# mjrgh/DCSExplorer

Measured on AMD Instinct MI355X. Metric: bit_exact_int16_pcm_samples_per_sec, higher is better.
Workload: dtype int16; 1 GPU; survey3_65536; gpu_max_hw_queues=4, samples_per_frame=240, frames_per_wave=8, wavefronts_per_launch=8192, arithmetic=ADSP-2105 1.15 fixed point, 32-bit integer intermediates, partition=range over streams, no collective, scale=1, inflight=1, frames_per_chunk=all, full=False

## Files before the change

### dcsexplorer_amd/csrc/dcs_common.h

```cpp
#pragma once
#include <stdint.h>
#include <stddef.h>
#include "../../include/dcs_hip.h"

#define DCS_CB94_TOTAL   940
#define DCS_TRIE94_MAX   64
#define DCS_TRIE93_MAX   128

struct DcsLdsTables
{
    uint16_t cb94[DCS_CB94_TOTAL];
    uint16_t fast93[256];
    uint16_t trie93[DCS_TRIE93_MAX];
    uint16_t bandBits93a[64];
    uint16_t scaleCb93a[80];
    uint8_t  inputs93a[24];
    uint16_t raw94[20];
    uint32_t band94[72];
    uint16_t scale64[64];
    uint8_t  padDecode_[8];
    uint16_t cbInfo[8];
    uint16_t xlat94[48];
    uint8_t  preAdj94[32];
    uint16_t scaleMant[4];
    uint8_t  pad_[8];
};
#define DCS_LDS_DECODE_BYTES 3424
#define DCS_B94_RAW      (1u << 21)
#define DCS_B94_ZERO     (1u << 22)
#define DCS_B94_STOP     (1u << 23)
#define DCS_B94_FATAL    (1u << 24)
#define DCS_B94_TYPE0    51

#define DCS_LANE_CONSTS 24
#define DCS_K94_PRE   0
#define DCS_K94_TWB   8
#define DCS_K94_OVLA  22
#define DCS_K94_OVLB  23
#define DCS_K93_TWB   0
#define DCS_K93_OVL   15

struct DcsDevTables
{
    DcsLdsTables lds;
    uint32_t lane94[64][DCS_LANE_CONSTS];
    uint32_t lane93[64][DCS_LANE_CONSTS];
    uint16_t fast94[256];
    uint16_t trie94[DCS_TRIE94_MAX];
    uint16_t pair93a[2048];
    uint16_t fftCoef[256];
    uint16_t ovlCoef[16];
    int32_t  twA[8][4];
    uint8_t  multi94[6][1 << 10];
};
#define DCS_IDX_MULTI_BITS 10
#define DCS_IDX_MULTI_SAMPLES 4

const DcsDevTables &dcsTables();

int dcsFrameScaleV(const uint16_t *vol, uint16_t *mixMul, const uint8_t *counted, int nch);

#define DCS_POOL_DW_PER_FRAME 56
#define DCS_POOL_DW_MIN       320
#define DCS_MAX_FRAME_BITS    4480

#ifdef __cplusplus
static inline
#ifdef __HIPCC__
__host__ __device__
#endif
uint32_t dcsPoolDwords(uint64_t streamOff, uint32_t hdrLen, uint32_t bitOff, uint32_t nBits)
{
    const uint32_t inDword = static_cast<uint32_t>(((streamOff + 2 + hdrLen) * 8 + bitOff) & 31);
    return (inDword + nBits + 31) / 32 + 3;
}
#endif

#ifdef __cplusplus
static inline
#ifdef __HIPCC__
__host__ __device__
#endif
constexpr uint32_t dcsPoolCapacity(int fpw)
{
    return static_cast<uint32_t>(fpw * DCS_POOL_DW_PER_FRAME > DCS_POOL_DW_MIN ? fpw * DCS_POOL_DW_PER_FRAME : DCS_POOL_DW_MIN);
}
#endif

#define DCS_SLOT_HALO      0x01u
#define DCS_SLOT_EXT_TAIL  0x02u
#define DCS_SLOT_EXPORT    0x04u
#define DCS_SLOT_IMPORT    0x08u
#define DCS_SLOT_KEEP_TAIL 0x10u
#define DCS_SLOT_EMPTY     0x80u
#define DCS_NO_PREV_SLOT   0xFFu

struct DcsSlot
{
    uint32_t job;
    uint8_t  prevSlot;
    uint8_t  flags;
    uint8_t  nSrc;
    uint8_t  shiftXform;
    uint32_t firstSrc;
    uint32_t prevJob;
    uint32_t runStartDw;
    uint16_t runNDw;
// ... 177 lines not shown
```

### dcsexplorer_amd/csrc/dcs_decode_chunk.inc.h

```cpp
    DCS_STAMP(1);

    struct { uint32_t job; uint32_t prevSlot, flags, nSrc, shiftXform; uint32_t firstSrc, prevJob, poolOff, bpl; } slot;
    uint32_t exportNext;
    uint4 pd0, pd1, phdr;
    uint2 pd2;
    {
        uint4 *scratch = reinterpret_cast<uint4 *>(L.pool());
        static_assert(kHeadVec * 16 <= poolDwords(FPW) * 4, "the package head fits in the bit pool");
        if (lane < kHeadVec)
            scratch[lane] = phead0;
        if (kHeadLoads > 1 && lane + 64 < kHeadVec)
            scratch[lane + 64] = phead1;
        waveSync();
        const uint4 *sp5 = scratch + 5 * s;
        const uint4 s0 = sp5[0];
        pd0 = sp5[1]; pd1 = sp5[2];
        const uint4 d2v = sp5[3];
        pd2 = make_uint2(d2v.x, d2v.y);
        phdr = sp5[4];
        waveSync();
        slot.job = s0.x;
        slot.prevSlot = s0.y & 0xFFu; slot.flags = (s0.y >> 8) & 0xFFu; slot.nSrc = (s0.y >> 16) & 0xFFu; slot.shiftXform = s0.y >> 24;
        slot.firstSrc = s0.z; slot.prevJob = s0.w;
        slot.poolOff = d2v.z & 0xFFFFu;
        slot.bpl = (d2v.z >> 16) & 0xFFu;
        const unsigned long long exportSlots = __ballot(lane < FPW && !(slot.flags & DCS_SLOT_EMPTY) && (slot.flags & DCS_SLOT_EXPORT) != 0);
        exportNext = static_cast<uint32_t>(__builtin_amdgcn_readlane(static_cast<int>(d2v.w), exportSlots != 0 ? static_cast<int>(__builtin_ctzll(exportSlots)) : 0));
    }

    const int firstXform = __builtin_amdgcn_readfirstlane(static_cast<int>(slot.shiftXform >> 4)) == DCS_XFORM_94 ? DCS_XFORM_94 : DCS_XFORM_93;
    if (PASS == 0 || firstXform != constsXform)
    {
        constsXform = firstXform;
        loadLaneConsts(a.tables, lane, constsXform, C);
    }
#pragma unroll
    for (int t = 0 ; t < kPoolPieces ; ++t)
    {
        const int i = lane * 4 + 256 * t;
        const bool in = i < imgDw;
        if (i < poolDwords(FPW))
            ldsWrite4(L.pool() + i, in ? pimg[t].x : 0u, in ? pimg[t].y : 0u, in ? pimg[t].z : 0u, in ? pimg[t].w : 0u);
    }

    const bool live = !(slot.flags & DCS_SLOT_EMPTY);
    struct { uint32_t firstSrc; int nSrc; int volShift; int xform; uint32_t prev; } job;
    job.firstSrc = slot.firstSrc; job.nSrc = slot.nSrc; job.volShift = slot.shiftXform & 15;
    job.xform = slot.shiftXform >> 4; job.prev = slot.prevJob;

    uint32_t err = 0;
    {
        uint32_t *pool = L.pool();
        const DcsLdsTables *T = L.tables();
        uint16_t *row = L.row(s);
        const uint32_t *blobW = reinterpret_cast<const uint32_t *>(a.blob);
        const uint32_t blobWords = static_cast<uint32_t>((a.blobLen + 3) >> 2);
        const int myNSrc = live ? job.nSrc : 0;

        auto unpackRound = [&](auto r0tag, const int r)
        {
            constexpr bool R0 = decltype(r0tag)::value;
            const bool has = r < myNSrc;
            const uint4 *sdp = reinterpret_cast<const uint4 *>(&a.srcs[has ? job.firstSrc + r : 0]);
            uint4 d0 = make_uint4(0, 0, 0, 0), d1 = d0;
            uint2 d2 = make_uint2(0, 0);
            uint2 sp = make_uint2(0, 0);
            const int bplSlot = slot.bpl;
            if (R0)
            {
                if (has) { d0 = pd0; d1 = pd1; d2 = pd2; sp = psplit; }
            }
            else if (has) { d0 = sdp[0]; d1 = sdp[1]; d2 = *reinterpret_cast<const uint2 *>(sdp + 2); }
            const uint64_t streamOff = static_cast<uint64_t>(d0.x) | (static_cast<uint64_t>(d0.y) << 32);
            const uint32_t mixMul = d0.z & 0xFFFFu;
            const int format = static_cast<int>((d0.z >> 16) & 0xFFu);
            const int hdrLen = has ? static_cast<int>(d0.z >> 24) : 16;
            const uint32_t bitOff = d0.w;
            const uint32_t nBits = d1.x & 0xFFFFu, hdrBits = d1.x >> 16;
            const int nBands = static_cast<int>((d2.y >> 16) & 0xFFu);
            const uint32_t flags = d2.y >> 24;
// ... 120 lines not shown
                    Q.nb = max((q == SUB - 1 ? nbEnd : nextBase) - myBase, 0);
                    if (SUB == 16)
                    {
                        const bool mid = format >= DCS_FMT_94_T0 && q == SUB - 1 && myBase == 15 && (sp.y & (DCS_SPLIT_MID15 << 16)) != 0;
                        const bool nextMid = __shfl(static_cast<int>(mid), lane + FPW) != 0;
                        Q.midStart = mid;
                        Q.midStraddle = mid && (sp.y & (DCS_MID15_STRADDLE << 16)) != 0;
                        Q.midEnd = q == SUB - 2 && nextMid;
                        if (Q.midEnd)
                            Q.nb = 16 - myBase;
                    }
                }
                else
                {
                    const int bpl = max((nb16 + SUB - 1) / SUB, 1);
                    if (format == DCS_FMT_93A_T1)
                    {
                        Q.bandBase = min(q * bpl, nb16);
                        Q.nb = min(max(nb16 - Q.bandBase, 0), bpl);
                    }
                    else
                    {
                        Q.bandBase = dcsLaneFirstBand(format, q, bpl, nb16);
                        Q.nb = (q == SUB - 1 ? nb16 : dcsLaneFirstBand(format, q + 1, bpl, nb16)) - Q.bandBase;
                    }
                }
                if (q != 0 && Q.nb != 0)
                {
                    if (!R0)
                        sp = reinterpret_cast<const uint2 *>(sdp)[5 + Q.bandBase - 1];
                    const uint32_t sp0 = sp.x, sp1 = sp.y;
                    relBits = sp0 & 0x7FFFu;
                    Q.prv = sp0 >> 16;
                    Q.prvDelta = sp1 & 0xFFFFu;
                    const uint32_t st = sp1 >> 16;
                    Q.outIdx = static_cast<int>(st & 0x1FFu);
                    Q.subType = static_cast<int>((st >> 9) & 3u);
                    Q.reuse = (st & 0x800u) != 0;
                    Q.first = false;
                }
            }
            const uint32_t inPool = static_cast<uint32_t>(bitPos & 31) + relBits;
            const uint32_t *brAt = pool + (ok ? off + (inPool >> 5) : 0u);
            const int brBit = static_cast<int>(inPool & 31);

            if (R0) DCS_STAMP(12);
            const bool is94 = ok && format >= DCS_FMT_94_T0;
            const bool is93a = ok && format == DCS_FMT_93A_T1 && Q.nb != 0 && !(Q.bandBase != 0 && Q.reuse);
            const bool is93 = ok && format < DCS_FMT_93A_T1;
            if (__any(is94))
            {
                BR94 br;
                br.init(brAt, brBit);
                err |= unpack94<R0, BR94, SUB>(T, row, br, Q, format, mixMul, is94, stamp);
            }
            BR93 br;
            br.init(brAt, brBit);
            if (__any(is93))
                err |= unpack93<R0, BR93>(T, row, br, Q, format, mixMul, is93, stamp);
            if (is93a)
            {
                constexpr bool kSpreadTail = SUB == 16 && !R0;
                const int end = Q.bandBase + Q.nb;
                const int end2 = (!R0 && SUB != 16 && end >= 16 && nBands > 16) ? nBands : end;
                const int prv0 = Q.bandBase == 0 ? 0x1A : sx16(Q.prv), out0 = Q.bandBase == 0 ? 0 : Q.outIdx;
                const int hb0 = static_cast<int>(Q.h0 & 0xFFu);
                if (pairTableInLds(FPW))
                    err |= unpack93a<R0, BR93>(T, row, br, hb0, mixMul, reinterpret_cast<const uint16_t *>(smem + ldsBytes(FPW) - 4096),
                                         Q.bandBase, end2, prv0, out0);
                else
                    err |= unpack93a<R0, BR93>(T, row, br, hb0, mixMul, a.tables->pair93a, Q.bandBase, end2, prv0, out0);
                if (kSpreadTail && pairTableInLds(FPW) && q < 2 && 16 + q < nBands)
                {
                    const uint32_t r0 = q == 0 ? Q.t0 : Q.t2, r1 = q == 0 ? Q.t1 : Q.t3;
                    if (!((r1 >> 16) & 0x800u))
                    {
                        const uint32_t inPool2 = static_cast<uint32_t>(bitPos & 31) + (r0 & 0xFFFFu);
                        BR93 br2;
                        br2.init(pool + off + (inPool2 >> 5), static_cast<int>(inPool2 & 31));
                        err |= unpack93a<R0, BR93>(T, row, br2, hb0, mixMul, reinterpret_cast<const uint16_t *>(smem + ldsBytes(FPW) - 4096),
                                             16 + q, 17 + q, sx16(r0 >> 16), static_cast<int>((r1 >> 16) & 0x1FFu));
                    }
                }
            }
            waveSync();
        };

        {
            if (__any(myNSrc > 0))
                unpackRound(std::true_type{}, 0);
            for (int r = 1 ; __any(r < myNSrc) ; ++r)
                unpackRound(std::false_type{}, r);
        }

        DCS_STAMP(4);
        if (__any(err != 0))
        {
#pragma unroll
            for (int m = FPW ; m < 64 ; m <<= 1)
                err |= __shfl_xor(err, m);
        }
        if (live && q == 0)
        {
            if (job.xform == DCS_XFORM_93)
                dcMagnitude93(row);
            if (!(slot.flags & DCS_SLOT_HALO) && a.err != nullptr)
                a.err[slot.job] = err;
// ... 191 lines not shown
```

### dcsexplorer_amd/csrc/dcs_kernels.hip.h

```cpp
#pragma once
#include <hip/hip_runtime.h>
#include <type_traits>
#include <cstddef>
#include "dcs_common.h"

namespace dcsk {

struct Stamper
{
#ifdef DCS_STAMPS
    unsigned long long *p;
#ifdef DCS_STAMPS_REALTIME
    __device__ __forceinline__ void operator()(int k) const { if (p != nullptr) p[k] = __builtin_amdgcn_s_memrealtime(); }
#else
    __device__ __forceinline__ void operator()(int k) const { if (p != nullptr) p[k] = __builtin_amdgcn_s_memtime(); }
#endif
#else
    __device__ __forceinline__ void operator()(int) const { }
#endif
};
#define DCS_STAMP(k) stamp(k)

__device__ __forceinline__ unsigned long long handoffWord(uint32_t epoch, uint32_t who, uint32_t payload)
{
    return (static_cast<unsigned long long>(epoch) << 33) | (static_cast<unsigned long long>(who) << 32) | payload;
}
__device__ __forceinline__ bool handoffMeets(unsigned long long old, uint32_t epoch, uint32_t whoWanted)
{
    return static_cast<uint32_t>(old >> 32) == ((epoch << 1) | whoWanted);
}
constexpr int kWavesPerBlock = 4;
#ifndef DCS_ROW_BYTES
#define DCS_ROW_BYTES 528
#endif
constexpr int kRowBytes = DCS_ROW_BYTES;

__host__ __device__ constexpr int poolDwords(int fpw) { return static_cast<int>(dcsPoolCapacity(fpw)); }
__host__ __device__ constexpr int subLanes(int fpw) { return 64 / fpw; }

__host__ __device__ constexpr int waveLdsBytes(int fpw) { return fpw * kRowBytes + (fpw + 1) * 32 + poolDwords(fpw) * 4; }
__host__ __device__ constexpr bool pairTableInLds(int fpw) { return fpw <= 8; }
__host__ __device__ constexpr int ldsBytes(int fpw)
{
    return DCS_LDS_DECODE_BYTES + kWavesPerBlock * waveLdsBytes(fpw) + (pairTableInLds(fpw) ? 4096 : 0);
}

__device__ __forceinline__ int sx16(uint32_t v) { return static_cast<int>(static_cast<int16_t>(v)); }

__device__ __forceinline__ int sat16(int v) { return min(max(v, -32768), 32767); }

__device__ __forceinline__ uint32_t prodSS(int a, int b) { return static_cast<uint32_t>(__mul24(a, b)) << 1; }

__device__ __forceinline__ int roundHi(uint32_t mr, int lastProdUndoubled)
{
    mr += 0x8000u;
    if ((lastProdUndoubled & 0x7FFF) == 0x4000)
        mr &= ~0x10000u;
    return static_cast<int>(mr) >> 16;
}

__device__ __forceinline__ void rotate(int are, int aim, int c, int s, int &tre, int &tim)
{
    const int p1 = __mul24(are, c), p2 = __mul24(aim, s);
    tre = roundHi(static_cast<uint32_t>(p1 - p2) << 1, p2);
    const int q1 = __mul24(aim, c), q2 = __mul24(are, s);
    tim = roundHi(static_cast<uint32_t>(q1 + q2) << 1, q2);
}

__device__ __forceinline__ int calcExp32(uint32_t x)
{
    const uint32_t y = (static_cast<int>(x) < 0) ? ~x : x;
    int n = (y == 0) ? 32 : __clz(static_cast<int>(y));
    n -= 1;
    if (n > 31) n = 31;
    return -n;
}

typedef const uint32_t __attribute__((address_space(3))) *LdsDwordPtr;
struct BitReader
{
    static constexpr bool kDirect = false;
    uint32_t pa;
    uint32_t hi, lo;
    int negpos;

    __device__ __forceinline__ void init(const uint32_t *pool, int bitInDword)
    {
        hi = 0;
        lo = pool[0];
        pa = static_cast<uint32_t>(reinterpret_cast<uintptr_t>((LdsDwordPtr)(pool + 1)));
        negpos = 0;
        skip(bitInDword);
    }
    __device__ __forceinline__ uint32_t cur() const { return __builtin_amdgcn_alignbit(hi, lo, static_cast<uint32_t>(negpos)); }
    __device__ __forceinline__ uint32_t peek(int n) const { return cur() >> (32 - n); }
    __device__ __forceinline__ uint32_t prefetch() const { return *reinterpret_cast<LdsDwordPtr>(static_cast<uintptr_t>(pa)); }
    __device__ __forceinline__ void skip(int n, uint32_t ahead)
    {
        negpos -= n;
        const bool refill = negpos < 0;
        hi = refill ? lo : hi;
        lo = refill ? ahead : lo;
        const uint32_t sign = static_cast<uint32_t>(negpos) >> 31;
        asm("v_lshl_add_u32 %0, %1, 2, %0" : "+v"(pa) : "v"(sign));
        negpos &= 31;
    }
    __device__ __forceinline__ void skipTight(uint32_t n, uint32_t ahead)
    {
        uint32_t t;
        asm("v_sub_co_u32 %3, vcc, %3, %5\n\t"
            "v_cndmask_b32 %0, %0, %1, vcc\n\t"
            "v_cndmask_b32 %1, %1, %6, vcc\n\t"
            "v_lshrrev_b32 %4, 31, %3\n\t"
            "v_lshl_add_u32 %2, %4, 2, %2\n\t"
            "v_and_b32 %3, 31, %3"
            : "+v"(hi), "+v"(lo), "+v"(pa), "+v"(negpos), "=&v"(t)
            : "v"(n), "v"(ahead)
            : "vcc");
    }
    __device__ __forceinline__ void skip(int n) { skip(n, prefetch()); }
    __device__ __forceinline__ uint32_t get(int n) { const uint32_t v = peek(n); skip(n); return v; }
    __device__ __forceinline__ uint32_t bitAddr() const { return (pa - 4u) * 8u - static_cast<uint32_t>(negpos); }
    __device__ __forceinline__ void initAt(uint32_t bits)
    {
        init((const uint32_t *)reinterpret_cast<LdsDwordPtr>(static_cast<uintptr_t>((bits >> 5) << 2)), static_cast<int>(bits & 31u));
    }
};

struct DirectReader
{
    static constexpr bool kDirect = true;
    uint32_t bp;

    __device__ __forceinline__ void init(const uint32_t *pool, int bitInDword)
    {
        bp = static_cast<uint32_t>(reinterpret_cast<uintptr_t>((LdsDwordPtr)pool)) * 8u + static_cast<uint32_t>(bitInDword) - 1u;
    }
    __device__ __forceinline__ uint32_t cur() const
    {
        const LdsDwordPtr w = reinterpret_cast<LdsDwordPtr>(static_cast<uintptr_t>((bp >> 3) & ~3u));
        return __builtin_amdgcn_alignbit(w[0], w[1], ~bp);
    }
    __device__ __forceinline__ uint32_t peek(int n) const { return cur() >> (32 - n); }
    __device__ __forceinline__ uint32_t prefetch() const { return 0u; }
    __device__ __forceinline__ void skip(int n) { bp += static_cast<uint32_t>(n); }
    __device__ __forceinline__ void skip(int n, uint32_t) { skip(n); }
    __device__ __forceinline__ void skipTight(uint32_t n, uint32_t) { bp += n; }
    __device__ __forceinline__ uint32_t get(int n) { const uint32_t v = peek(n); skip(n); return v; }
    __device__ __forceinline__ uint32_t bitAddr() const { return bp + 1u; }
    __device__ __forceinline__ void initAt(uint32_t bits) { bp = bits - 1u; }
};

template <class BR>
__device__ __forceinline__ int readVlc(BR &br, const uint16_t *fast, const uint16_t *trie)
{
    uint32_t e = fast[br.peek(8)];
    if (e & 0x8000)
    {
        br.skip(static_cast<int>((e >> 8) & 0xF));
        return static_cast<int>(e & 0xFF);
    }
    br.skip(8);
    uint32_t w = br.cur();
    int n = 0;
    do
    {
        e = trie[e + (w >> 31)];
        w <<= 1;
        ++n;
    }
    while (!(e & 0x8000) && n < 24);
    br.skip(n);
    return static_cast<int>(e & 0xFF);
}

template <int FPW>
struct Lds
{
    unsigned char *tab;
    unsigned char *base;
    unsigned char *poolBase;
    __device__ __forceinline__ const DcsLdsTables *tables() const { return reinterpret_cast<const DcsLdsTables *>(tab); }
    __device__ __forceinline__ uint16_t *row(int s) const { return reinterpret_cast<uint16_t *>(base + s * kRowBytes); }
    __device__ __forceinline__ uint16_t *tails() const { return reinterpret_cast<uint16_t *>(base + FPW * kRowBytes); }
    __device__ __forceinline__ uint32_t *pool() const { return reinterpret_cast<uint32_t *>(poolBase); }
};

struct Quarter
{
    uint32_t h0, h1, h2, h3;
    uint32_t t0, t1, t2, t3;
    int bandBase;
    int nb;
    int outIdx;
    uint32_t preAdj;
    uint32_t prv, prvDelta;
    int subType;
    bool reuse, first;
    bool midEnd, midStart, midStraddle;
};

__device__ __forceinline__ int byteOf(uint32_t w0, uint32_t w1, uint32_t w2, uint32_t w3, int b)
{
    const int i = b >> 2;
    const uint32_t lo = (i & 1) ? w1 : w0, hi = (i & 1) ? w3 : w2;
    const uint32_t w = (i & 2) ? hi : lo;
    return static_cast<int>((w >> (8 * (b & 3))) & 0xFFu);
}

__device__ __forceinline__ int mul24(int a, int b)
{
    int r;
    asm("v_mul_i32_i24 %0, %1, %2" : "=v"(r) : "v"(a), "v"(b));
    return r;
}

template <bool FIRST>
__device__ __forceinline__ void mixAdd(uint16_t *cell, int scaledProduct, uint32_t mixMul)
{
    uint32_t t, acc;
    asm("v_mul_i32_i24_sdwa %0, sext(%1), %2 dst_sel:DWORD dst_unused:UNUSED_PAD src0_sel:WORD_0 src1_sel:DWORD"
        : "=v"(t) : "v"(scaledProduct), "v"(mixMul));
    asm("v_add_u32_sdwa %0, %1, %2 dst_sel:DWORD dst_unused:UNUSED_PAD src0_sel:DWORD src1_sel:WORD_0"
        : "=v"(acc) : "v"(t), "v"(scaledProduct));
    if (!FIRST)
        acc += static_cast<uint32_t>(*cell) << 16;
    *cell = static_cast<uint16_t>(acc >> 16);
}
typedef uint16_t __attribute__((address_space(3))) *LdsWordPtr;
template <bool FIRST>
__device__ __forceinline__ void mixAddAt(uint32_t cellAddr, int scaledProduct, uint32_t mixMul)
{
    const LdsWordPtr cell = reinterpret_cast<LdsWordPtr>(static_cast<uintptr_t>(cellAddr));
    uint32_t t, acc;
    asm("v_mul_i32_i24_sdwa %0, sext(%1), %2 dst_sel:DWORD dst_unused:UNUSED_PAD src0_sel:WORD_0 src1_sel:DWORD"
        : "=v"(t) : "v"(scaledProduct), "v"(mixMul));
    asm("v_add_u32_sdwa %0, %1, %2 dst_sel:DWORD dst_unused:UNUSED_PAD src0_sel:DWORD src1_sel:WORD_0"
        : "=v"(acc) : "v"(t), "v"(scaledProduct));
// ... 5 lines not shown
__device__ __forceinline__ uint32_t mixAddCarry(uint16_t *cell, int scaledProduct, uint32_t mixMul, uint32_t addLow)
{
    uint32_t t, acc;
    asm("v_mul_i32_i24_sdwa %0, sext(%1), %2 dst_sel:DWORD dst_unused:UNUSED_PAD src0_sel:WORD_0 src1_sel:DWORD"
        : "=v"(t) : "v"(scaledProduct), "v"(mixMul));
    asm("v_add_u32_sdwa %0, %1, %2 dst_sel:DWORD dst_unused:UNUSED_PAD src0_sel:DWORD src1_sel:WORD_0"
        : "=v"(acc) : "v"(t), "v"(addLow));
    if (!FIRST)
        acc += static_cast<uint32_t>(*cell) << 16;
    *cell = static_cast<uint16_t>(acc >> 16);
    return acc;
}
template <bool FIRST>
__device__ __forceinline__ uint32_t mixAddCarryAt(uint32_t cellAddr, int scaledProduct, uint32_t mixMul, uint32_t addLow)
{
    const LdsWordPtr cell = reinterpret_cast<LdsWordPtr>(static_cast<uintptr_t>(cellAddr));
    uint32_t t, acc;
    asm("v_mul_i32_i24_sdwa %0, sext(%1), %2 dst_sel:DWORD dst_unused:UNUSED_PAD src0_sel:WORD_0 src1_sel:DWORD"
        : "=v"(t) : "v"(scaledProduct), "v"(mixMul));
    asm("v_add_u32_sdwa %0, %1, %2 dst_sel:DWORD dst_unused:UNUSED_PAD src0_sel:DWORD src1_sel:WORD_0"
        : "=v"(acc) : "v"(t), "v"(addLow));
    if (!FIRST)
        acc += static_cast<uint32_t>(*cell) << 16;
    *cell = static_cast<uint16_t>(acc >> 16);
    return acc;
}
__device__ __forceinline__ int mulLowWord(uint32_t x, int y)
{
    int r;
    asm("v_mul_i32_i24_sdwa %0, sext(%1), %2 dst_sel:DWORD dst_unused:UNUSED_PAD src0_sel:WORD_0 src1_sel:DWORD" : "=v"(r) : "v"(x), "v"(y));
    return r;
}
__device__ __forceinline__ void mixSub(uint16_t *cell, int scaledProduct, uint32_t mixMul)
{
    const uint32_t s = static_cast<uint32_t>(scaledProduct) & 0xFFFFu;
    const uint32_t c = (s + static_cast<uint32_t>(__mul24(sx16(s), static_cast<int>(mixMul)))) >> 16;
    *cell = static_cast<uint16_t>(*cell - c);
}

__device__ __forceinline__ uint32_t scaleFactor(const DcsLdsTables *T, int code)
{
    return T->scale64[code & 63];
}

__device__ __forceinline__ void dcFixup(uint16_t *row, uint32_t saved1)
{
    const int delta = sat16(sx16(row[1]) - sx16(saved1));
    row[0] = static_cast<uint16_t>(sat16(delta + sx16(row[0])));
    row[1] = static_cast<uint16_t>(saved1);
}

constexpr int kDummyWord = 256;

template <bool FIRST, class BR, int SUB>
__device__ uint32_t unpack94(const DcsLdsTables *T, uint16_t *row, BR &br, const Quarter &Q,
                             int format, uint32_t mixMul, bool has, const Stamper &stamp)
{
    const bool type1 = format != DCS_FMT_94_T0;
    uint32_t err = 0;
    int nb = has ? Q.nb : 0;
    const int b1 = Q.bandBase + nb;
    const int before = Q.bandBase <= 0 ? 0 : Q.bandBase == 1 ? 7 : 15 + 16 * (Q.bandBase - 2);
    const int upTo = b1 <= 0 ? 0 : b1 == 1 ? 7 : b1 >= 16 ? 255 : 15 + 16 * (b1 - 2);
    const int midAdvance = 16 - (Q.midStraddle ? 1 + static_cast<int>((Q.h3 >> 30) & 1u) : 0);
    int outIdx = min(Q.outIdx, 256 - ((SUB == 16 && Q.midStart) ? midAdvance : upTo - before));
    bool valid = true;
    const bool owner = has && Q.bandBase == 0;
    const uint32_t saved1 = (owner && !FIRST) ? row[1] : 0u;

    stamp(8);
    int k = 0;
    const int keyLim = type1 ? 16 : 17;
    uint32_t cell = static_cast<uint32_t>(reinterpret_cast<uintptr_t>((LdsWordPtr)row)) + 2u * static_cast<uint32_t>(outIdx);
    uint32_t cellEnd = cell;
    uint32_t cellStart = cell;
    uint32_t startBits = 0;
    const uint16_t *book = T->cb94;
    int shPeek = 0, shIdx = 0, scale = 0;
    uint32_t incSh = 1;
    uint32_t valOff = 0, valWidth = 8;
    for (int round = 0 ; ; ++round)
    {
        if (SUB == 16 && Q.midEnd && cell > cellEnd)
            cellEnd = cell;
        if (cell > cellEnd)
        {
            cell -= 1u << incSh;
            if (valid)
            {
                BR r2;
                r2.initAt(startBits);
                uint32_t c2 = cellStart;
                while (c2 + (1u << incSh) < cellEnd)
                {
                    const uint32_t e = book[r2.cur() >> shIdx];
                    r2.skip(static_cast<int>((e >> 8) & 0x1F));
                    const uint32_t step = e >> 13;
                    if (step == 1)
                        mixSub((uint16_t *)reinterpret_cast<LdsWordPtr>(static_cast<uintptr_t>(c2)),
                               mul24(static_cast<int>(static_cast<int8_t>(e & 0xFF)), scale), mixMul);
                    c2 += step << incSh;
                }
            }
            valid = false; err |= DCS_FRAME_STOP;
            cellEnd = cell;
        }
        const bool start = cell == cellEnd && k < nb;
        if (!__any(start || cell < cellEnd))
            break;
        if (start)
        {
            const int band = Q.bandBase + k;
            ++k;
            const int hb = byteOf(Q.h0, Q.h1, Q.h2, Q.h3, band) & 0x7F;
            const int code0 = byteOf(Q.t0, Q.t1, Q.t2, Q.t3, band);
            const int cls = band < 3 ? 0 : band < 6 ? 17 : 34;
            const int key = min(code0, keyLim) + (type1 ? cls : DCS_B94_TYPE0);
            const uint32_t e = T->band94[key];
            const int count0 = band < 2 ? 7 + band : band == 15 ? 32 : 16;
            const uint32_t strided = (static_cast<uint32_t>(hb) >> 6) & 1u;
            const uint32_t count = static_cast<uint32_t>(count0) >> strided;
            incSh = 1u + strided;
            const int pre = (type1 && band < 3) ? static_cast<int>((Q.preAdj >> (4 * band)) & 15u) : 0;
            scale = static_cast<int>(scaleFactor(T, hb + pre + static_cast<int>(e >> 25)));
            book = reinterpret_cast<const uint16_t *>(T) + (e & 0x7FFu);
            shPeek = static_cast<int>((e >> 11) & 31u);
            shIdx = static_cast<int>((e >> 16) & 31u);
            const bool isRaw = (e & DCS_B94_RAW) != 0;
            valOff = isRaw ? static_cast<uint32_t>(shPeek) : 0u;
            valWidth = isRaw ? 32u - static_cast<uint32_t>(shPeek) : 8u;
            const bool zeroBand = (e & DCS_B94_ZERO) != 0, fatal = (e & DCS_B94_FATAL) != 0;
            uint32_t i = (e & (DCS_B94_ZERO | DCS_B94_FATAL)) == 0 ? count : 0u;
            if (SUB == 16 && band == 15 && i != 0)
            {
                if (Q.midEnd) i = count - (count >> 1);
                if (Q.midStart) i = (count >> 1) - (Q.midStraddle ? 1u : 0u);
            }
            cell += zeroBand ? 2u * count : 0u;
            if (fatal)
            {
                err |= DCS_FRAME_FATAL | DCS_FRAME_STOP;
                nb = 0;
            }
            if (!valid)
                scale = 0;
            cellStart = cell;
            cellEnd = cell + (i << incSh);
            startBits = br.bitAddr();
        }

        if (round == 0) stamp(9);
        const uint32_t roundLen = round == 0 ? 7u : round == 1 ? 9u : 16u;
        const uint32_t roundEnd = min(cellEnd, cell + (roundLen << incSh));
        if (cell < roundEnd)
        {
            do
            {
                const uint32_t ahead = br.prefetch();
                const uint32_t w = br.cur();
                const uint32_t e = book[w >> shIdx];
                const int v = __builtin_amdgcn_sbfe(__builtin_amdgcn_perm(w, e, 0x07060100u), valOff, valWidth);
                const uint32_t step = e >> 13;
                br.skipTight((e >> 8) & 0x1Fu, ahead);
// ... 704 lines not shown
    for (int r = 0 ; r < 16 ; ++r)
        x[r] = y[r];
    DCS_XSTAMP(10);
    DCS_PACE_STEP(1);
    stageB<false, 8, 4>(x, C.k + DCS_K93_TWB, R);
    stageB<false, 4, 3>(x, C.k + DCS_K93_TWB + 1, R);
    DCS_PACE_STEP(2);
    stageB<false, 2, 2>(x, C.k + DCS_K93_TWB + 3, R);
    stageB<false, 1, 1>(x, C.k + DCS_K93_TWB + 7, R);
    DCS_XSTAMP(11);
    if (__any(P.shiftPair != 0))
    {
#pragma unroll
        for (int r = 0 ; r < 16 ; ++r)
            x[r] = pkAshr(x[r], P.shiftPair);
    }
}

#ifndef DCS_CPW2_SCHED
#define DCS_CPW2_SCHED 1
#endif
struct PaceSchedule { int entry; bool steps; int levels; };
__host__ __device__ constexpr PaceSchedule paceSchedule(int cpw, int pass)
{
    if (cpw == 1)
        return { 3, true, kPaceSteps };
#if DCS_CPW2_SCHED == 0
    return pass == 0 ? PaceSchedule{ 3, false, kPaceSteps } : PaceSchedule{ 3, true, 2 | (1 << 2) | (0 << 4) };
#elif DCS_CPW2_SCHED == 1
    return pass == 0 ? PaceSchedule{ 3, false, kPaceSteps } : PaceSchedule{ 2, true, 1 | (1 << 2) | (0 << 4) };
#elif DCS_CPW2_SCHED == 2
    return pass == 0 ? PaceSchedule{ 3, true, 3 | (3 << 2) | (2 << 4) } : PaceSchedule{ 2, true, 1 | (1 << 2) | (0 << 4) };
#else
    return pass == 0 ? PaceSchedule{ 3, true, 3 | (2 << 2) | (2 << 4) } : PaceSchedule{ 1, true, 1 | (0 << 2) | (0 << 4) };
#endif
}

template <int FPW, int CPW = 1>
#ifndef DCS_MIN_WAVES
#define DCS_MIN_WAVES 4
#endif
__global__ void __launch_bounds__(64 * kWavesPerBlock, DCS_MIN_WAVES)
dcsDecodeKernel(uint8_t *kPackages, const DcsDevTables *kTables, uint32_t kNChunks, uint32_t kFlags, uint32_t kEpoch, uint32_t kNJobs,
                int16_t *kPcm, unsigned long long *kHandoff, uint32_t *kErr, int16_t *kTailsOut,
                const uint8_t *kBlob, uint64_t kBlobLen, const DcsSrcDesc *kSrcs, const int16_t *kTailsIn, unsigned long long *kDebug)
{
    DcsKernelArgs a;
    a.blob = kBlob; a.blobLen = kBlobLen; a.srcs = kSrcs; a.packages = kPackages; a.nChunks = kNChunks; a.nJobs = kNJobs;
    a.pcm = kPcm; a.err = kErr; a.tailsIn = kTailsIn; a.tailsOut = kTailsOut; a.tables = kTables; a.debug = kDebug;
    a.handoff = kHandoff; a.epoch = kEpoch; a.flags = kFlags;
    extern __shared__ __attribute__((aligned(16))) unsigned char smem[];
    const int wave = static_cast<int>(threadIdx.x) >> 6;
    const int lane = static_cast<int>(threadIdx.x) & 63;
    constexpr int kPoolBytes = poolDwords(FPW) * 4, kTileBytes = FPW * kRowBytes + (FPW + 1) * 32;
    static_assert(kPoolBytes % 16 == 0 && kWavesPerBlock * kTileBytes >= 8192, "LDS layout");
    const Lds<FPW> L{ smem, smem + DCS_LDS_DECODE_BYTES + kWavesPerBlock * kPoolBytes + wave * kTileBytes,
                      smem + DCS_LDS_DECODE_BYTES + wave * kPoolBytes };
    uint32_t blk = blockIdx.x;
    if (a.flags & DCS_BATCH_XCD_RANGES)
        blk = (blk & 7u) * (gridDim.x >> 3) + (blk >> 3);
    static_assert(CPW == 1 || CPW == 2, "one or two chunks per wavefront");
    const uint32_t wv = blk * kWavesPerBlock + static_cast<uint32_t>(wave);
    const uint32_t nFirst = CPW == 2 ? (a.nChunks + 1u) >> 1 : a.nChunks;
    auto stamperOf = [&](uint32_t chunk, bool valid)
    {
#ifdef DCS_STAMPS
        return Stamper{ (lane == 0 && a.debug != nullptr && valid) ? a.debug + static_cast<size_t>(chunk) * 16 : nullptr };
#else
        return Stamper{};
#endif
    };
    {
        const Stamper stamp = stamperOf(wv, wv < nFirst);
        DCS_STAMP(0);
    }
    const bool pacedLaunch = (a.flags & DCS_BATCH_PACED) != 0;
    const bool paced = pacedLaunch && blockIdx.x + ((a.flags >> DCS_BATCH_CUS8_SHIFT) & 0xFFu) * 32u >= gridDim.x;
    if (pacedLaunch) __builtin_amdgcn_s_setprio(3);
    constexpr int SUB = subLanes(FPW);
#ifndef DCS_DIRECT_MAX_FPW
#define DCS_DIRECT_MAX_FPW 4
#endif
    using BR94 = typename std::conditional<(FPW <= DCS_DIRECT_MAX_FPW), DirectReader, BitReader>::type;
    using BR93 = DirectReader;
    static_assert(SUB * FPW == 64 && SUB <= 16, "every lane unpacks; a frame has at most 16 split lanes");
    const int s = lane % FPW;
    const int q = lane / FPW;
    const bool unpacker = q < SUB;

    const uint32_t layout = (a.flags >> DCS_BATCH_IMG_SHIFT) & DCS_BATCH_IMG_MASK;
    const int imgDw = static_cast<int>(dcsPkgImgDw(layout));
    const bool split4 = (layout & DCS_PKG_SPLIT4) != 0;
    const uint32_t offPool = split4 ? dcsPkgOffPool(FPW, DCS_PKG_SPLIT4) : dcsPkgOffPool(FPW, 0);
    constexpr int kHeadVec = FPW * 5, kHeadLoads = (kHeadVec + 63) / 64;
    static_assert(kHeadLoads <= 2, "package head: two 16-byte loads per lane at most");
    uint4 phead0, phead1 = make_uint4(0, 0, 0, 0);
    uint2 psplit;
    constexpr int kPoolPieces = (poolDwords(FPW) + 255) / 256;
    uint4 pimg[kPoolPieces];
    {
        const uint32_t chunk = wv;
        const bool valid = wv < nFirst;
#include "dcs_request_package.inc.h"
    }
    TwA W;
    loadTwA(a.tables, W);

    {
        constexpr int kTableVec = DCS_LDS_DECODE_BYTES / 16;
        static_assert(kTableVec <= 64 * kWavesPerBlock, "one piece of the tables per thread");
        const uint4 piece = reinterpret_cast<const uint4 *>(&a.tables->lds)[min(static_cast<int>(threadIdx.x), kTableVec - 1)];
        const bool stagePairs = pairTableInLds(FPW) && (a.flags & DCS_BATCH_HAS_93A_T1);
        uint4 pairPiece = make_uint4(0, 0, 0, 0);
        if (stagePairs)
            pairPiece = reinterpret_cast<const uint4 *>(a.tables->pair93a)[threadIdx.x];
        uint4 *tile = reinterpret_cast<uint4 *>(L.base);
#ifndef DCS_CLEAR_FIRST_MAX_FPW
#define DCS_CLEAR_FIRST_MAX_FPW 8
#endif
        constexpr bool kClearFirst = FPW <= DCS_CLEAR_FIRST_MAX_FPW;
        if (kClearFirst)
            for (int i = lane ; i < FPW * kRowBytes / 16 ; i += 64)
                tile[i] = make_uint4(0, 0, 0, 0);
        if (static_cast<int>(threadIdx.x) < kTableVec)
            reinterpret_cast<uint4 *>(smem)[threadIdx.x] = piece;
        if (stagePairs)
            reinterpret_cast<uint4 *>(smem + ldsBytes(FPW) - 4096)[threadIdx.x] = pairPiece;
        if (!kClearFirst)
            for (int i = lane ; i < FPW * kRowBytes / 16 ; i += 64)
                tile[i] = make_uint4(0, 0, 0, 0);
    }
    __syncthreads();
    if (wv >= nFirst)
        return;

    int constsXform = -1;
    LaneConsts C;
    if constexpr (CPW == 1)
    {
        constexpr int PASS = 0;
        constexpr PaceSchedule kPace = paceSchedule(CPW, PASS);
        const uint32_t chunk = wv;
        const Stamper stamp = stamperOf(chunk, true);
#include "dcs_decode_chunk.inc.h"
    }
    else
    {
        auto decodeChunk = [&](const uint32_t chunk, auto passTag)
        {
            constexpr int PASS = decltype(passTag)::value;
            constexpr PaceSchedule kPace = paceSchedule(CPW, PASS);
            const Stamper stamp = stamperOf(chunk, true);
#include "dcs_decode_chunk.inc.h"
        };
        decodeChunk(wv, std::integral_constant<int, 0>{});
        const uint32_t second = wv + nFirst;
        if (second < a.nChunks)
        {
            {
                const Stamper stamp0 = stamperOf(second, true);
                stamp0(0);
            }
            constexpr PaceSchedule kPace = paceSchedule(CPW, 1);
            if (paced && kPace.entry != 3) __builtin_amdgcn_s_setprio(kPace.entry);
            {
                const uint32_t chunk = second;
                const bool valid = true;
#include "dcs_request_package.inc.h"
            }
            uint4 *tile = reinterpret_cast<uint4 *>(L.base);
            for (int i = lane ; i < FPW * kRowBytes / 16 ; i += 64)
                tile[i] = make_uint4(0, 0, 0, 0);
            waveSync();
            decodeChunk(second, std::integral_constant<int, 1>{});
// ... 6 lines not shown
```

### dcsexplorer_amd/csrc/dcs_tables.cpp

```cpp
#include <cstddef>
#include "dcs_common.h"
#include "dcs_tables.h"
#include <stdlib.h>
#include <string.h>
#include <vector>

namespace {

template <size_t N, typename F>
void buildVlc(const DcsVlc (&codes)[N], uint16_t *fast, uint16_t *trie, size_t trieCap, F payload)
{
    struct Node { int child[2]; int leaf; };
    std::vector<Node> nodes;
    nodes.push_back({{-1, -1}, -1});
    for (const DcsVlc &c : codes)
    {
        int n = 0;
        for (int b = c.len - 1 ; b >= 0 ; --b)
        {
            int bit = (c.code >> b) & 1;
            if (nodes[n].child[bit] < 0)
            {
                nodes[n].child[bit] = static_cast<int>(nodes.size());
                nodes.push_back({{-1, -1}, -1});
// ... 85 lines not shown
            uint32_t at = 0, samples = 0;
            for (;;)
            {
                const uint32_t idx = ((x << at) & ((1u << DCS_IDX_MULTI_BITS) - 1)) >> (DCS_IDX_MULTI_BITS - maxBits[k]);
                const uint32_t e = book[idx], len = (e >> 8) & 0x1F, step = (e >> 13) == 2 ? 2 : 1;
                if (len == 0 || at + len > DCS_IDX_MULTI_BITS || samples + step > DCS_IDX_MULTI_SAMPLES)
                    break;
                at += len;
                samples += step;
            }
            if (at == 0 || samples == 0)
                abort();
            t.multi94[k - 1][x] = static_cast<uint8_t>(at | (samples << 4));
        }
    }
    for (int w = 7 ; w <= 16 ; ++w)
        t.lds.raw94[2 * (w - 7)] = t.lds.raw94[2 * (w - 7) + 1] = static_cast<uint16_t>((w << 8) | (1 << 13));

    buildVlc(kVlc94BandTypeDelta, t.fast94, t.trie94, DCS_TRIE94_MAX, [](int v) { return v + 16; });
    buildVlc(kVlc93BandType, t.lds.fast93, t.lds.trie93, DCS_TRIE93_MAX, [](int v) { return v; });

    for (int i = 0 ; i < 16 ; ++i)
    {
        t.lds.xlat94[i] = kXlatB02[i];
        t.lds.xlat94[16 + i] = kXlatB35[i];
        t.lds.xlat94[32 + i] = kXlatB6F[i];
        t.lds.preAdj94[i] = kPreAdjSub0[i];
        t.lds.preAdj94[16 + i] = kPreAdjSub3[i];
    }
    for (int k = 0 ; k < 72 ; ++k)
    {
        const bool type1 = k < DCS_B94_TYPE0;
        const int cls = type1 ? k / 17 : 0, code0 = type1 ? k % 17 : k - DCS_B94_TYPE0;
        if (k > DCS_B94_TYPE0 + 17)
            continue;
        const uint32_t x = t.lds.xlat94[cls * 16 + (code0 & 15)];
        const bool fatal1 = type1 && code0 > 15;
        const int code = (type1 && !fatal1) ? static_cast<int>(x & 0xFF) : code0;
        const uint32_t adj = type1 ? x >> 8 : 0;
        const bool zero = code0 == 0;
        const bool fatal = !zero && (fatal1 || code > 16);
        const bool stop = !zero && !fatal && code == 0;
        const bool raw = code > 6;
        const uint32_t info = t.lds.cbInfo[code < 7 ? code : 7];
        const uint32_t shPeek = 32u - (raw ? static_cast<uint32_t>(code < 16 ? code : 16) : (info & 0xF));
        const uint32_t shIdx = raw ? 31u : shPeek;
        const size_t book = raw ? offsetof(DcsLdsTables, raw94) / 2 + 2 * static_cast<size_t>((code < 16 ? code : 16) - 7)
                                : offsetof(DcsLdsTables, cb94) / 2 + (info >> 4);
        if (book > 0x7FF || adj > 0x7F || stop)
            abort();
        t.lds.band94[k] = static_cast<uint32_t>(book) | ((shPeek & 31u) << 11) | ((shIdx & 31u) << 16) | (raw ? DCS_B94_RAW : 0u)
                        | (zero ? DCS_B94_ZERO : 0u) | (stop ? DCS_B94_STOP : 0u) | (fatal ? DCS_B94_FATAL : 0u) | (adj << 25);
    }
    memcpy(t.lds.bandBits93a, kBandBits93a, sizeof(t.lds.bandBits93a));
    memcpy(t.lds.scaleCb93a, kScaleCb93a, sizeof(t.lds.scaleCb93a));
    for (int i = 0 ; i < 18 ; ++i)
        t.lds.inputs93a[i] = kInputsPerBand93a[i];
    memcpy(t.lds.scaleMant, kScaleMant, sizeof(t.lds.scaleMant));
    for (int c = 0 ; c < 64 ; ++c)
        t.lds.scale64[c] = static_cast<uint16_t>(kScaleMant[c & 3] >> (15 - ((c >> 2) & 15)));
    if (kScaleMant[0] != 0x8000 || kScaleMant[1] != 0x9838 || kScaleMant[2] != 0xB505 || kScaleMant[3] != 0xD745)
        abort();
    memcpy(t.pair93a, kPair93a, sizeof(t.pair93a));
    memcpy(t.fftCoef, kFftCoef, sizeof(t.fftCoef));
    if (kFftCoef[0x80] != 0x8000 || kFftCoef[0] != 0x0000 || kFftCoef[0x81] != 0x0000 || kFftCoef[1] != 0x8000)
        abort();
    memcpy(t.ovlCoef, kOverlapCoef, sizeof(t.ovlCoef));
    static const int kTwAInKernel[8][2] = { { -65536, 0 }, { 0, -65536 }, { -46340, -46340 }, { 46340, -46340 },
                                            { -60548, -25080 }, { 25080, -60548 }, { -25080, -60548 }, { 60548, -25080 } };
    for (int k = 0 ; k < 8 ; ++k)
    {
        const int c = static_cast<int16_t>(kFftCoef[0x80 + k]), sn = static_cast<int16_t>(kFftCoef[k]);
        t.twA[k][0] = 2 * c; t.twA[k][1] = 2 * sn; t.twA[k][2] = -2 * sn; t.twA[k][3] = 0;
        if (kTwAInKernel[k][0] != 2 * c || kTwAInKernel[k][1] != 2 * sn)
            abort();
    }

    auto rev = [](int v, int bits) { int r = 0; for (int i = 0 ; i < bits ; ++i) r |= ((v >> i) & 1) << (bits - 1 - i); return r; };
    auto tw = [&](int part) { return static_cast<uint32_t>(kFftCoef[0x80 + part]) | (static_cast<uint32_t>(kFftCoef[part]) << 16); };
    for (int lane = 0 ; lane < 64 ; ++lane)
    {
        uint32_t *k94 = t.lane94[lane], *k93 = t.lane93[lane];
        const int l8 = lane & 7, l16 = lane & 15;
        for (int j = 0 ; j < 8 ; ++j)
        {
            const int i = l8 + 8 * j;
            k94[DCS_K94_PRE + j] = static_cast<uint32_t>(kFftCoef[rev(2 + 4 * i, 9)]) | (static_cast<uint32_t>(kFftCoef[rev(4 * i, 9)]) << 16);
        }
        for (int k = 0 ; k < 2 ; ++k) k94[DCS_K94_TWB + k] = tw(2 * l8 + k);
        for (int k = 0 ; k < 4 ; ++k) k94[DCS_K94_TWB + 2 + k] = tw(4 * l8 + k);
        for (int k = 0 ; k < 8 ; ++k) k94[DCS_K94_TWB + 6 + k] = tw(8 * l8 + k);
        k93[DCS_K93_TWB] = tw(l16);
        for (int k = 0 ; k < 2 ; ++k) k93[DCS_K93_TWB + 1 + k] = tw(2 * l16 + k);
        for (int k = 0 ; k < 4 ; ++k) k93[DCS_K93_TWB + 3 + k] = tw(4 * l16 + k);
        for (int k = 0 ; k < 8 ; ++k) k93[DCS_K93_TWB + 7 + k] = tw(8 * l16 + k);
        const int m = rev(l8, 3);
        k94[DCS_K94_OVLA] = static_cast<uint32_t>(kOverlapCoef[2 * m]) | (static_cast<uint32_t>(kOverlapCoef[2 * m + 1]) << 16);
        k94[DCS_K94_OVLB] = static_cast<uint32_t>(kOverlapCoef[15 - 2 * m]) | (static_cast<uint32_t>(kOverlapCoef[14 - 2 * m]) << 16);
        const int i = rev(l16, 4);
        k93[DCS_K93_OVL] = static_cast<uint32_t>(kOverlapCoef[i]) | (static_cast<uint32_t>(kOverlapCoef[15 - i]) << 16);
    }
    return t;
}

}

const DcsDevTables &dcsTables()
{
    static const DcsDevTables tables = build();
    return tables;
}

static_assert(sizeof(DcsLdsTables) % 16 == 0, "LDS table block must be a multiple of 16 bytes");
static_assert(DCS_LDS_DECODE_BYTES % 16 == 0 && DCS_LDS_DECODE_BYTES == offsetof(DcsLdsTables, cbInfo), "the decode kernel stages the block up to the index walk's tables");
static_assert(offsetof(DcsDevTables, lane94) % 16 == 0 && offsetof(DcsDevTables, lane93) % 16 == 0 && offsetof(DcsDevTables, twA) % 16 == 0, "lane constants and twiddles are fetched as uint4");
static_assert(sizeof(DcsSrcDesc) == 160, "DcsSrcDesc layout");
static_assert(offsetof(DcsSrcDesc, idx) == 12, "DcsSrcDesc layout");
static_assert(sizeof(DcsFrameJob) == 16, "DcsFrameJob layout");
static_assert(sizeof(DcsFrameIndex) == 148 && offsetof(DcsFrameIndex, split) == 28, "DcsFrameIndex layout");
static_assert(sizeof(DcsSlot) == 32, "DcsSlot layout");
static_assert(offsetof(DcsDevTables, pair93a) % 4 == 0, "OS93a sample pairs are read as 32-bit words");
```

Baseline: 507.3 billion samples/s.

## Precompute per-band 94 decode plans in LDS before the unpack loop

Adds a host-built template table of per-band codebook, shift, width and span records, staged into LDS for FPW=8. At frame start each lane builds the per-band plan records from the header bytes, so the first-quarter unpack94 loop reads a compact 8-byte record per band instead of redoing the band-table decode and scale lookup serially. This adds LDS per wave, but a static assert keeps workgroups per CU unchanged. It also adds an extra plan-building pass and changes how the bit reader is re-seeked.

```diff
diff --git a/dcsexplorer_amd/csrc/dcs_common.h b/dcsexplorer_amd/csrc/dcs_common.h
--- a/dcsexplorer_amd/csrc/dcs_common.h
+++ b/dcsexplorer_amd/csrc/dcs_common.h
@@ -52,7 +52,9 @@
     uint16_t ovlCoef[16];
     int32_t  twA[8][4];
     uint8_t  multi94[6][1 << 10];
-};
+    uint32_t plan94[2][72][2];
+};
+#define DCS_PLAN94_BYTES 1152
 #define DCS_IDX_MULTI_BITS 10
 #define DCS_IDX_MULTI_SAMPLES 4
 
diff --git a/dcsexplorer_amd/csrc/dcs_decode_chunk.inc.h b/dcsexplorer_amd/csrc/dcs_decode_chunk.inc.h
--- a/dcsexplorer_amd/csrc/dcs_decode_chunk.inc.h
+++ b/dcsexplorer_amd/csrc/dcs_decode_chunk.inc.h
@@ -4,6 +4,7 @@
     uint32_t exportNext;
     uint4 pd0, pd1, phdr;
     uint2 pd2;
+    uint32_t planHdr0 = 0, planHdr1 = 0, planType0 = 0, planType1 = 0;
     {
         uint4 *scratch = reinterpret_cast<uint4 *>(L.pool());
         static_assert(kHeadVec * 16 <= poolDwords(FPW) * 4, "the package head fits in the bit pool");
@@ -18,6 +19,12 @@
         const uint4 d2v = sp5[3];
         pd2 = make_uint2(d2v.x, d2v.y);
         phdr = sp5[4];
+        if constexpr (bandPlanInLds(FPW))
+        {
+            const unsigned char *bytes = reinterpret_cast<const unsigned char *>(sp5) + q;
+            planType0 = bytes[36]; planType1 = bytes[44];
+            planHdr0 = bytes[64]; planHdr1 = bytes[72];
+        }
         waveSync();
         slot.job = s0.x;
         slot.prevSlot = s0.y & 0xFFu; slot.flags = (s0.y >> 8) & 0xFFu; slot.nSrc = (s0.y >> 16) & 0xFFu; slot.shiftXform = s0.y >> 24;
@@ -26,6 +33,22 @@
         slot.bpl = (d2v.z >> 16) & 0xFFu;
         const unsigned long long exportSlots = __ballot(lane < FPW && !(slot.flags & DCS_SLOT_EMPTY) && (slot.flags & DCS_SLOT_EXPORT) != 0);
         exportNext = static_cast<uint32_t>(__builtin_amdgcn_readlane(static_cast<int>(d2v.w), exportSlots != 0 ? static_cast<int>(__builtin_ctzll(exportSlots)) : 0));
+    }
+
+    if constexpr (bandPlanInLds(FPW))
+    {
+        const int fmt0 = static_cast<int>((pd0.z >> 16) & 0xFFu);
+        if (__any(!(slot.flags & DCS_SLOT_EMPTY) && slot.nSrc != 0 && fmt0 >= DCS_FMT_94_T0))
+        {
+            uint2 *plan = reinterpret_cast<uint2 *>(L.plan());
+            const uint2 *tmpl = reinterpret_cast<const uint2 *>(smem + planTableOffset(FPW));
+            const bool type1 = fmt0 != DCS_FMT_94_T0;
+            const uint32_t keyLim = type1 ? 16u : 17u;
+            const uint32_t cls0 = !type1 ? DCS_B94_TYPE0 : q < 3 ? 0u : q < 6 ? 17u : 34u, cls1 = type1 ? 34u : DCS_B94_TYPE0;
+            const uint32_t pre = (type1 && q < 3) ? (pd2.y >> (4 * q)) & 15u : 0u;
+            plan[lane] = planBand94(L.tables(), tmpl, planHdr0, planType0, cls0, keyLim, q < 2 ? 7u + q : 16u, pre);
+            plan[lane + 64] = planBand94(L.tables(), tmpl, planHdr1, planType1, cls1, keyLim, q == 7 ? 32u : 16u, 0u);
+        }
     }
 
     const int firstXform = __builtin_amdgcn_readfirstlane(static_cast<int>(slot.shiftXform >> 4)) == DCS_XFORM_94 ? DCS_XFORM_94 : DCS_XFORM_93;
@@ -252,7 +275,10 @@
             {
                 BR94 br;
                 br.init(brAt, brBit);
-                err |= unpack94<R0, BR94, SUB>(T, row, br, Q, format, mixMul, is94, stamp);
+                const uint32_t planAt = (R0 && bandPlanInLds(FPW))
+                    ? static_cast<uint32_t>(reinterpret_cast<uintptr_t>((LdsBytePtr)L.plan())) + static_cast<uint32_t>(Q.bandBase * FPW + s) * kPlanRecBytes
+                    : 0u;
+                err |= unpack94<R0, BR94, SUB>(T, row, br, Q, format, mixMul, is94, stamp, planAt);
             }
             BR93 br;
             br.init(brAt, brBit);
diff --git a/dcsexplorer_amd/csrc/dcs_kernels.hip.h b/dcsexplorer_amd/csrc/dcs_kernels.hip.h
--- a/dcsexplorer_amd/csrc/dcs_kernels.hip.h
+++ b/dcsexplorer_amd/csrc/dcs_kernels.hip.h
@@ -38,12 +38,20 @@
 __host__ __device__ constexpr int poolDwords(int fpw) { return static_cast<int>(dcsPoolCapacity(fpw)); }
 __host__ __device__ constexpr int subLanes(int fpw) { return 64 / fpw; }
 
-__host__ __device__ constexpr int waveLdsBytes(int fpw) { return fpw * kRowBytes + (fpw + 1) * 32 + poolDwords(fpw) * 4; }
+constexpr int kPlanRecBytes = 8;
+__host__ __device__ constexpr bool bandPlanInLds(int fpw) { return fpw == 8; }
+__host__ __device__ constexpr int planBytes(int fpw) { return bandPlanInLds(fpw) ? 16 * fpw * kPlanRecBytes : 0; }
+__host__ __device__ constexpr int waveTileBytes(int fpw) { return fpw * kRowBytes + (fpw + 1) * 32 + planBytes(fpw); }
+__host__ __device__ constexpr int waveLdsBytes(int fpw) { return waveTileBytes(fpw) + poolDwords(fpw) * 4; }
 __host__ __device__ constexpr bool pairTableInLds(int fpw) { return fpw <= 8; }
 __host__ __device__ constexpr int ldsBytes(int fpw)
 {
-    return DCS_LDS_DECODE_BYTES + kWavesPerBlock * waveLdsBytes(fpw) + (pairTableInLds(fpw) ? 4096 : 0);
-}
+    return DCS_LDS_DECODE_BYTES + kWavesPerBlock * waveLdsBytes(fpw) + (bandPlanInLds(fpw) ? DCS_PLAN94_BYTES : 0) + (pairTableInLds(fpw) ? 4096 : 0);
+}
+__host__ __device__ constexpr int planTableOffset(int fpw) { return ldsBytes(fpw) - (pairTableInLds(fpw) ? 4096 : 0) - DCS_PLAN94_BYTES; }
+__host__ __device__ constexpr int ldsAllocBytes(int fpw) { return (ldsBytes(fpw) + 1279) / 1280 * 1280; }
+static_assert(4 * ldsAllocBytes(4) <= 163840 && 4 * ldsAllocBytes(8) <= 163840 && 3 * ldsAllocBytes(16) <= 163840,
+              "workgroups per compute unit: the band plan must not cost one");
 
 __device__ __forceinline__ int sx16(uint32_t v) { return static_cast<int>(static_cast<int16_t>(v)); }
 
@@ -125,6 +133,8 @@
     {
         init((const uint32_t *)reinterpret_cast<LdsDwordPtr>(static_cast<uintptr_t>((bits >> 5) << 2)), static_cast<int>(bits & 31u));
     }
+    __device__ __forceinline__ uint32_t mark() const { return (pa << 3) | static_cast<uint32_t>(negpos); }
+    __device__ __forceinline__ void initAtMark(uint32_t m) { initAt((m & ~31u) - 32u - (m & 31u)); }
 };
 
 struct DirectReader
@@ -149,6 +159,8 @@
     __device__ __forceinline__ uint32_t get(int n) { const uint32_t v = peek(n); skip(n); return v; }
     __device__ __forceinline__ uint32_t bitAddr() const { return bp + 1u; }
     __device__ __forceinline__ void initAt(uint32_t bits) { bp = bits - 1u; }
+    __device__ __forceinline__ uint32_t mark() const { return bitAddr(); }
+    __device__ __forceinline__ void initAtMark(uint32_t m) { initAt(m); }
 };
 
 template <class BR>
@@ -184,6 +196,7 @@
     __device__ __forceinline__ uint16_t *row(int s) const { return reinterpret_cast<uint16_t *>(base + s * kRowBytes); }
     __device__ __forceinline__ uint16_t *tails() const { return reinterpret_cast<uint16_t *>(base + FPW * kRowBytes); }
     __device__ __forceinline__ uint32_t *pool() const { return reinterpret_cast<uint32_t *>(poolBase); }
+    __device__ __forceinline__ unsigned char *plan() const { return base + FPW * kRowBytes + (FPW + 1) * 32; }
 };
 
 struct Quarter
@@ -295,10 +308,24 @@
 
 constexpr int kDummyWord = 256;
 
+typedef uint8_t __attribute__((address_space(3))) *LdsBytePtr;
+__device__ __forceinline__ uint2 planBand94(const DcsLdsTables *T, const uint2 *tmpl, uint32_t hdrByte, uint32_t typeByte,
+                                            uint32_t cls, uint32_t keyLim, uint32_t count0, uint32_t pre)
+{
+    const uint32_t strided = (hdrByte >> 6) & 1u;
+    const uint2 t = tmpl[min(typeByte, keyLim) + (strided * 72u + cls)];
+    const uint32_t scale = scaleFactor(T, static_cast<int>(hdrByte + pre + ((t.x >> 16) & 0x7Fu)));
+    const uint32_t book = static_cast<uint32_t>(reinterpret_cast<uintptr_t>((LdsWordPtr)reinterpret_cast<const uint16_t *>(T))) + (t.x & 0xFFFFu);
+    const uint32_t span = static_cast<uint32_t>(__mul24(static_cast<int>(count0 >> strided), static_cast<int>(t.x >> 24)));
+    return make_uint2(book | (scale << 16), t.y | (span << 24));
+}
+
 template <bool FIRST, class BR, int SUB>
 __device__ uint32_t unpack94(const DcsLdsTables *T, uint16_t *row, BR &br, const Quarter &Q,
-                             int format, uint32_t mixMul, bool has, const Stamper &stamp)
-{
+                             int format, uint32_t mixMul, bool has, const Stamper &stamp, uint32_t planAt = 0)
+{
+    constexpr bool kPlan = FIRST && SUB == 8;
+    constexpr uint32_t kPlanBandBytes = kPlanRecBytes * 8;
     const bool type1 = format != DCS_FMT_94_T0;
     uint32_t err = 0;
     int nb = has ? Q.nb : 0;
@@ -313,6 +340,7 @@
 
     stamp(8);
     int k = 0;
+    uint32_t planEnd = planAt + kPlanBandBytes * static_cast<uint32_t>(nb);
     const int keyLim = type1 ? 16 : 17;
     uint32_t cell = static_cast<uint32_t>(reinterpret_cast<uintptr_t>((LdsWordPtr)row)) + 2u * static_cast<uint32_t>(outIdx);
     uint32_t cellEnd = cell;
@@ -332,7 +360,10 @@
             if (valid)
             {
                 BR r2;
-                r2.initAt(startBits);
+                if (kPlan)
+                    r2.initAtMark(startBits);
+                else
+                    r2.initAt(startBits);
                 uint32_t c2 = cellStart;
                 while (c2 + (1u << incSh) < cellEnd)
                 {
@@ -348,10 +379,36 @@
             valid = false; err |= DCS_FRAME_STOP;
             cellEnd = cell;
         }
-        const bool start = cell == cellEnd && k < nb;
+        const bool start = cell == cellEnd && (kPlan ? planAt < planEnd : k < nb);
         if (!__any(start || cell < cellEnd))
             break;
-        if (start)
+        if constexpr (kPlan)
+        {
+            if (start)
+            {
+                const LdsBytePtr rec = reinterpret_cast<LdsBytePtr>(static_cast<uintptr_t>(planAt));
+                planAt += kPlanBandBytes;
+                const uint32_t bookAt = *reinterpret_cast<LdsWordPtr>(rec);
+                const uint32_t recScale = *reinterpret_cast<LdsWordPtr>(rec + 2);
+                const uint32_t recOff = rec[5], recWidth = rec[6], span = rec[7];
+                shIdx = rec[4];
+                book = (const uint16_t *)reinterpret_cast<LdsWordPtr>(static_cast<uintptr_t>(bookAt));
+                valOff = recOff;
+                valWidth = recWidth;
+                incSh = __builtin_amdgcn_ubfe(recOff, 5u, 2u);
+                if (recOff > 0x7Fu)
+                {
+                    err |= DCS_FRAME_FATAL | DCS_FRAME_STOP;
+                    planEnd = 0;
+                }
+                scale = valid ? static_cast<int>(recScale) : 0;
+                cellEnd = cell + span;
+                cell = recWidth > 0x7Fu ? cellEnd : cell;
+                cellStart = cell;
+                startBits = br.mark();
+            }
+        }
+        else if (start)
         {
             const int band = Q.bandBase + k;
             ++k;
@@ -1162,7 +1219,7 @@
     extern __shared__ __attribute__((aligned(16))) unsigned char smem[];
     const int wave = static_cast<int>(threadIdx.x) >> 6;
     const int lane = static_cast<int>(threadIdx.x) & 63;
-    constexpr int kPoolBytes = poolDwords(FPW) * 4, kTileBytes = FPW * kRowBytes + (FPW + 1) * 32;
+    constexpr int kPoolBytes = poolDwords(FPW) * 4, kTileBytes = waveTileBytes(FPW);
     static_assert(kPoolBytes % 16 == 0 && kWavesPerBlock * kTileBytes >= 8192, "LDS layout");
     const Lds<FPW> L{ smem, smem + DCS_LDS_DECODE_BYTES + kWavesPerBlock * kPoolBytes + wave * kTileBytes,
                       smem + DCS_LDS_DECODE_BYTES + wave * kPoolBytes };
@@ -1225,11 +1282,20 @@
         if (stagePairs)
             pairPiece = reinterpret_cast<const uint4 *>(a.tables->pair93a)[threadIdx.x];
         uint4 *tile = reinterpret_cast<uint4 *>(L.base);
+        if constexpr (bandPlanInLds(FPW))
+        {
+            constexpr int kPlanVec = DCS_PLAN94_BYTES / 16;
+            const uint4 planPiece = reinterpret_cast<const uint4 *>(a.tables->plan94)[min(static_cast<int>(threadIdx.x), kPlanVec - 1)];
+            for (int i = lane ; i < FPW * kRowBytes / 16 ; i += 64)
+                tile[i] = make_uint4(0, 0, 0, 0);
+            if (static_cast<int>(threadIdx.x) < kPlanVec)
+                reinterpret_cast<uint4 *>(smem + planTableOffset(FPW))[threadIdx.x] = planPiece;
+        }
 #ifndef DCS_CLEAR_FIRST_MAX_FPW
 #define DCS_CLEAR_FIRST_MAX_FPW 8
 #endif
         constexpr bool kClearFirst = FPW <= DCS_CLEAR_FIRST_MAX_FPW;
-        if (kClearFirst)
+        if (kClearFirst && !bandPlanInLds(FPW))
             for (int i = lane ; i < FPW * kRowBytes / 16 ; i += 64)
                 tile[i] = make_uint4(0, 0, 0, 0);
         if (static_cast<int>(threadIdx.x) < kTableVec)
diff --git a/dcsexplorer_amd/csrc/dcs_tables.cpp b/dcsexplorer_amd/csrc/dcs_tables.cpp
--- a/dcsexplorer_amd/csrc/dcs_tables.cpp
+++ b/dcsexplorer_amd/csrc/dcs_tables.cpp
@@ -161,6 +161,19 @@
         t.lds.band94[k] = static_cast<uint32_t>(book) | ((shPeek & 31u) << 11) | ((shIdx & 31u) << 16) | (raw ? DCS_B94_RAW : 0u)
                         | (zero ? DCS_B94_ZERO : 0u) | (stop ? DCS_B94_STOP : 0u) | (fatal ? DCS_B94_FATAL : 0u) | (adj << 25);
     }
+    for (uint32_t strided = 0 ; strided < 2 ; ++strided)
+        for (int k = 0 ; k < 72 ; ++k)
+        {
+            const uint32_t e = t.lds.band94[k];
+            const uint32_t shPeek = (e >> 11) & 31u, shIdx = (e >> 16) & 31u;
+            const bool raw = (e & DCS_B94_RAW) != 0, zero = (e & DCS_B94_ZERO) != 0, fatal = (e & DCS_B94_FATAL) != 0;
+            const uint32_t valOff = raw ? shPeek : 0u, valWidth = raw ? 32u - shPeek : 8u;
+            const uint32_t perSample = fatal ? 0u : zero ? 2u : 2u << strided;
+            if (valWidth > 16 || (zero && fatal))
+                abort();
+            t.plan94[strided][k][0] = 2u * (e & 0x7FFu) | ((e >> 25) << 16) | (perSample << 24);
+            t.plan94[strided][k][1] = shIdx | ((valOff | ((1u + strided) << 5) | (fatal ? 0x80u : 0u)) << 8) | ((valWidth | (zero ? 0x80u : 0u)) << 16);
+        }
     memcpy(t.lds.bandBits93a, kBandBits93a, sizeof(t.lds.bandBits93a));
     memcpy(t.lds.scaleCb93a, kScaleCb93a, sizeof(t.lds.scaleCb93a));
     for (int i = 0 ; i < 18 ; ++i)
@@ -228,4 +241,5 @@
 static_assert(sizeof(DcsFrameJob) == 16, "DcsFrameJob layout");
 static_assert(sizeof(DcsFrameIndex) == 148 && offsetof(DcsFrameIndex, split) == 28, "DcsFrameIndex layout");
 static_assert(sizeof(DcsSlot) == 32, "DcsSlot layout");
+static_assert(offsetof(DcsDevTables, plan94) % 16 == 0 && sizeof(DcsDevTables::plan94) == DCS_PLAN94_BYTES, "the band plan's table is staged as uint4");
 static_assert(offsetof(DcsDevTables, pair93a) % 4 == 0, "OS93a sample pairs are read as 32-bit words");
```

Measured after the change: 513.7 billion samples/s (median of 6 runs). 1.01x the previous value.
